# junofficial/mppi_RobotArm

Measured on AMD Instinct MI355X. Metric: MPPI rollouts/sec (K×T state-steps/s) + control-step latency, K=65536 T=64, higher is better.
Workload: dtype f32

## Files before the change

### mppi_robotarm_amd/csrc/mppi_merge.h

```cpp
#pragma once

namespace mppi {


typedef unsigned int u32x2 __attribute__((__vector_size__(2 * sizeof(unsigned int))));
typedef unsigned int u32x4 __attribute__((__vector_size__(4 * sizeof(unsigned int))));
constexpr int kSC1 = 16;

__device__ __forceinline__ __amdgpu_buffer_rsrc_t rows_rsrc(const void* p, int bytes) {
    return __builtin_amdgcn_make_buffer_rsrc(const_cast<void*>(p), 0, bytes, 0x00020000);
}
__device__ __forceinline__ double ld_wt(__amdgpu_buffer_rsrc_t r, int idx) {
    return __builtin_bit_cast(double, __builtin_amdgcn_raw_buffer_load_b64(r, idx * 8, 0, kSC1));
}
__device__ __forceinline__ double ld_prev(__amdgpu_buffer_rsrc_t r, int idx) {
    return __builtin_bit_cast(double, __builtin_amdgcn_raw_buffer_load_b64(r, idx * 8, 0, 0));
}
__device__ __forceinline__ void st_wt(__amdgpu_buffer_rsrc_t r, int idx, double v) {
    __builtin_amdgcn_raw_buffer_store_b64(__builtin_bit_cast(u32x2, v), r, idx * 8, 0, kSC1);
}
constexpr int kOffRange = 1 << 26;

__device__ __forceinline__ void st_gran(__amdgpu_buffer_rsrc_t r, int idx, double v, unsigned tag) {
    const unsigned long long b = (unsigned long long)__double_as_longlong(v);
// ... 124 lines not shown
        } else {
            rho_r = ld_wt(rows, lrow);
            eta_l = ld_wt(rows, lrow + 1);
#pragma unroll
            for (int j = 0; j < LB; ++j) {
                const int i = j / MAXCH, col = tid + (j % MAXCH) * NT;
                v[j] = ld_wt(rows, (i < nr && col < ncol) ? (rb + i) * stride + 1 + col : kOffRange);
            }
        }
        const double rho_l = lane < nr ? rho_r : INFINITY;
        const double rnew = min_raw_f64(rho, wave_min_f64(rho_l));
        double s_l = 0.0;
        if (lane < nr) {
            const double s = exp((rnew - rho_l) * inv_lambda);
            s_l = s >= kMergeFloor ? s : 0.0;
        }
        const unsigned long long rel = __ballot(s_l != 0.0);
        const int nrr = __popcll(rel);
        nrel += nrr;
        if (rnew < rho && rho != INFINITY) {
            const double f = exp((rnew - rho) * inv_lambda);
#pragma unroll
            for (int ch = 0; ch < MAXCH; ++ch) acc[ch] *= f;
            eta *= f;
        }
        rho = rnew;
        if constexpr (EAGER) {
#pragma unroll
            for (int j = 0; j < LB; ++j) {
                const int i = j / MAXCH, ch = j % MAXCH;
                if (i < nr) {
                    const double s = readlane_f64(s_l, i);
                    if (s != 0.0) {
                        acc[ch] = fma(s, v[j], acc[ch]);
                        if (ch == 0) eta = fma(s, readlane_f64(eta_l, i), eta);
                    }
                }
            }
        } else {
            const int krow = lane < nrr ? select_bit(rel, lane) : 0;
            for (int b0 = 0; b0 < nrr; b0 += RB) {
                const bool eta_on = b0 == 0 && lane < nrr;
                const int eidx = eta_on ? (rb + krow) * stride + 1 : kOffRange;
                double x[LB];
                if constexpr (GRAN) {
                    u32x4 ge, gv[LB];
                    for (unsigned spins = 0;; ++spins) {
                        asm volatile("" ::: "memory");
                        ge = ld_gran(rows, eidx);
                        bool ok = !eta_on || gran_ok(ge, tag);
#pragma unroll
                        for (int j = 0; j < LB; ++j) {
                            const int i = b0 + j / MAXCH, col = tid + (j % MAXCH) * NT;
                            const bool on = i < nrr && col < ncol;
                            gv[j] = ld_gran(rows, on ? (rb + __builtin_amdgcn_readlane(krow, i)) * stride + 1 + col
                                                     : kOffRange);
                            ok = ok && (!on || gran_ok(gv[j], tag));
                        }
                        if (__all(ok)) break;
                        MPPI_SPIN_OR_GIVE_UP_L(spins, deadline, tmo, lane, gave_up = true);
                    }
                    if (eta_on) eta_l = gran_val(ge);
#pragma unroll
                    for (int j = 0; j < LB; ++j) x[j] = gran_val(gv[j]);
                } else {
                    if (b0 == 0) eta_l = ld_wt(rows, eidx);
#pragma unroll
                    for (int j = 0; j < LB; ++j) {
                        const int i = b0 + j / MAXCH, col = tid + (j % MAXCH) * NT;
                        x[j] = ld_wt(rows, (i < nrr && col < ncol)
                                               ? (rb + __builtin_amdgcn_readlane(krow, i)) * stride + 1 + col
                                               : kOffRange);
                    }
                }
#pragma unroll
                for (int j = 0; j < LB; ++j) {
                    const int i = b0 + j / MAXCH, ch = j % MAXCH;
                    if (i < nrr) {
                        const double s = readlane_f64(s_l, __builtin_amdgcn_readlane(krow, i));
                        acc[ch] = fma(s, x[j], acc[ch]);
                        if (ch == 0) eta = fma(s, readlane_f64(eta_l, i), eta);
                    }
                }
            }
        }
    }
    if (failed) *failed = __syncthreads_or(gave_up);
    if constexpr (final) {
        put_final<NT, MAXCH>(rho, acc, eta, nrel, geo, sm, out_row, w_eps_out);
    } else {
        auto put = [&](int col, double x) {
            if constexpr (GRAN) st_gran(*out_wt, out_idx * stride + col, x, tag);
            else st_wt(*out_wt, out_idx * stride + col, x);
        };
#pragma unroll
        for (int ch = 0; ch < MAXCH; ++ch) {
            const int col = tid + ch * NT;
            if (col >= ncol) continue;
            if (col == 0) put(0, rho);
            put(1 + col, acc[ch]);
        }
    }
}

template <int NT, int MAXCH, RowsVia VIA, class SM>
__device__ __forceinline__ bool direct_merge(__amdgpu_buffer_rsrc_t rows, int n, const RowGeo& geo,
                                             double inv_lambda, SM& sm, double* out_row, double* w_eps_out,
                                             unsigned tag, unsigned* tmo, unsigned long long* dbg = nullptr,
                                             const double* rho_pre = nullptr) {
    constexpr bool GRAN = VIA == RowsVia::Gran, PRE = VIA == RowsVia::Prev;
    constexpr int P = kDirectRows / 64;
    auto ld = [](__amdgpu_buffer_rsrc_t r, int idx) { return PRE ? ld_prev(r, idx) : ld_wt(r, idx); };
    constexpr int LB = 16;
    constexpr int RB = LB / MAXCH;
    const int tid = threadIdx.x, lane = tid & 63;
    const int stride = geo.stride, ncol = geo.ncol;
    double rho_l[P];
    if constexpr (GRAN) {
        if (tid < 64) {
            u32x4 gr[P];
            for (unsigned spins = 0;; ++spins) {
                asm volatile("" ::: "memory");
                bool ok = true;
#pragma unroll
                for (int j = 0; j < P; ++j) {
                    const int r = lane + 64 * j;
                    gr[j] = ld_gran(rows, r < n ? r * stride : kOffRange);
                    ok = ok && (r >= n || gran_ok(gr[j], tag));
                }
                if (__all(ok)) break;
                MPPI_SPIN_OR_GIVE_UP(spins, tmo, lane);
            }
#pragma unroll
            for (int j = 0; j < P; ++j) sm.rho[lane + 64 * j] = lane + 64 * j < n ? gran_val(gr[j]) : INFINITY;
        }
        __syncthreads();
#pragma unroll
        for (int j = 0; j < P; ++j) rho_l[j] = sm.rho[lane + 64 * j];
    } else if constexpr (PRE) {
#pragma unroll
        for (int j = 0; j < P; ++j) rho_l[j] = rho_pre[j];
    } else {
#pragma unroll
        for (int j = 0; j < P; ++j) {
            const int r = lane + 64 * j;
            const double x = ld_wt(rows, r < n ? r * stride : kOffRange);
            rho_l[j] = r < n ? x : INFINITY;
        }
    }
    double m = rho_l[0];
#pragma unroll
    for (int j = 1; j < P; ++j) m = min_raw_f64(m, rho_l[j]);
    const double rho = wave_min_f64(m);
    double s_l[P];
    unsigned long long rel[P];
    int nrel = 0;
#pragma unroll
    for (int j = 0; j < P; ++j) {
        const double s = exp((rho - rho_l[j]) * inv_lambda);
        s_l[j] = (lane + 64 * j < n && s >= kMergeFloor) ? s : 0.0;
        rel[j] = __ballot(s_l[j] != 0.0);
        nrel += __popcll(rel[j]);
    }
    const int G = MAXCH == 1 ? max(1, NT / ncol) : 1;
    if (nrel > (G > 1 ? min(64, 2 * kDirectMax * G) : kDirectMax)) return false;
    int k = lane, row = 0;
    bool found = false;
#pragma unroll
    for (int j = 0; j < P; ++j) {
        const int cnt = __popcll(rel[j]);
        if (!found && k < cnt) {
            row = 64 * j + select_bit(rel[j], k);
            found = true;
        } else if (!found) {
            k -= cnt;
        }
    }
    double sk = 0.0;
#pragma unroll
    for (int j = 0; j < P; ++j) {
        const double sj = __shfl(s_l[j], row & 63);
        if ((row >> 6) == j) sk = sj;
    }
    const bool mine = lane < nrel;
    STAMP(13, NOW());
    double acc[MAXCH], eta = 0.0, eta_k = 0.0;
#pragma unroll
    for (int ch = 0; ch < MAXCH; ++ch) acc[ch] = 0.0;
    if (G == 1) {
        for (int b0 = 0; b0 < nrel; b0 += RB) {
            double v[LB];
            if constexpr (GRAN) {
                const bool eta_on = b0 == 0 && mine;
                u32x4 ge, gv[LB];
                for (unsigned spins = 0;; ++spins) {
                    asm volatile("" ::: "memory");
                    ge = ld_gran(rows, eta_on ? row * stride + 1 : kOffRange);
                    bool ok = !eta_on || gran_ok(ge, tag);
#pragma unroll
                    for (int j = 0; j < LB; ++j) {
                        const int i = b0 + j / MAXCH, col = tid + (j % MAXCH) * NT;
                        const bool on = i < nrel && col < ncol;
                        gv[j] = ld_gran(rows, on ? __builtin_amdgcn_readlane(row, i) * stride + 1 + col : kOffRange);
                        ok = ok && (!on || gran_ok(gv[j], tag));
                    }
                    if (__all(ok)) break;
                    MPPI_SPIN_OR_GIVE_UP(spins, tmo, lane);
                }
                if (eta_on) eta_k = gran_val(ge);
#pragma unroll
                for (int j = 0; j < LB; ++j) v[j] = gran_val(gv[j]);
            } else {
                if (b0 == 0) eta_k = ld(rows, mine ? row * stride + 1 : kOffRange);
#pragma unroll
                for (int j = 0; j < LB; ++j) {
                    const int i = b0 + j / MAXCH, col = tid + (j % MAXCH) * NT;
                    v[j] = ld(rows, (i < nrel && col < ncol) ? __builtin_amdgcn_readlane(row, i) * stride + 1 + col
                                                              : kOffRange);
                }
            }
#pragma unroll
            for (int j = 0; j < LB; ++j) {
                const int i = b0 + j / MAXCH, ch = j % MAXCH;
                if (i < nrel) {
                    const double s = readlane_f64(sk, i);
                    acc[ch] = fma(s, v[j], acc[ch]);
                    if (ch == 0) eta = fma(s, readlane_f64(eta_k, i), eta);
                }
            }
        }
    } else {
        const int grp = tid / ncol, gcol = tid - grp * ncol;
        const bool active = grp < G;
        for (int b0 = 0; b0 < nrel; b0 += RB * G) {
            double v[LB], sf[LB];
            int roff[LB];
            bool on[LB];
#pragma unroll
            for (int j = 0; j < LB; ++j) {
                const int i = b0 + grp + G * j;
                on[j] = active && i < nrel;
                const int r = __builtin_amdgcn_ds_bpermute(min(i, 63) << 2, row);
                sf[j] = __shfl(sk, min(i, 63));
                roff[j] = on[j] ? r * stride + 1 + gcol : kOffRange;
            }
            if constexpr (GRAN) {
                u32x4 gv[LB];
                for (unsigned spins = 0;; ++spins) {
                    asm volatile("" ::: "memory");
                    bool ok = true;
#pragma unroll
                    for (int j = 0; j < LB; ++j) {
                        gv[j] = ld_gran(rows, roff[j]);
                        ok = ok && (!on[j] || gran_ok(gv[j], tag));
                    }
                    if (__all(ok)) break;
                    MPPI_SPIN_OR_GIVE_UP(spins, tmo, lane);
                }
#pragma unroll
                for (int j = 0; j < LB; ++j) v[j] = gran_val(gv[j]);
            } else {
#pragma unroll
                for (int j = 0; j < LB; ++j) v[j] = ld(rows, roff[j]);
            }
#pragma unroll
            for (int j = 0; j < LB; ++j)
                if (on[j]) acc[0] = fma(sf[j], v[j], acc[0]);
        }
        if (active) sm.part[tid] = acc[0];
        __syncthreads();
        if (grp == 0) {
            double a = sm.part[gcol];
            for (int g = 1; g < G; ++g) a += sm.part[g * ncol + gcol];
            acc[0] = a;
            if (tid == 0) sm.red[0] = a;
        }
        __syncthreads();
        eta = sm.red[0];
    }
    STAMP(14, NOW());
    put_final<NT, MAXCH>(rho, acc, eta, nrel, geo, sm, out_row, w_eps_out);
    return true;
}

__device__ __forceinline__ bool arrive_last(unsigned* counter, unsigned expected, unsigned* s_flag, bool acquire) {
    asm volatile("s_waitcnt vmcnt(0)" ::: "memory");
    __syncthreads();
    if (threadIdx.x == 0) {
        const unsigned prev = __hip_atomic_fetch_add(counter, 1u, __ATOMIC_RELAXED, __HIP_MEMORY_SCOPE_AGENT);
        const bool last = prev == expected - 1;
        if (last) __hip_atomic_store(counter, 0u, __ATOMIC_RELAXED, __HIP_MEMORY_SCOPE_AGENT);
        if (last && acquire) {
            __builtin_amdgcn_fence(__ATOMIC_ACQUIRE, "agent");
            asm volatile("s_waitcnt vmcnt(0)" ::: "memory");
        }
        *s_flag = last ? 1u : 0u;
    }
    __syncthreads();
    return *s_flag != 0;
}

template <int NT, int MAXCH, bool POLL, class SM>
__device__ __forceinline__ bool handoff_merge(__amdgpu_buffer_rsrc_t slab_r, __amdgpu_buffer_rsrc_t gslab_r, int nrows,
                                              const RowGeo& geo, double inv_lambda, SM& sm, unsigned* counters,
                                              bool acquire, unsigned* s_flag, double* partial_out, double* w_eps_out,
                                              unsigned tag, unsigned* epoch, unsigned* tmo, unsigned long long* dbg,
                                              unsigned long long* direct_dbg) {
    constexpr RowsVia VIA = POLL ? RowsVia::Gran : RowsVia::Wt;
    const int ngroups = (nrows + kGroup - 1) / kGroup;
    const int g = blockIdx.x / kGroup;
    const int gsz = min(kGroup, nrows - g * kGroup);
    if constexpr (POLL) {
        if ((int)blockIdx.x != g * kGroup) return false;
        STAMP(3, NOW());
        if (ngroups == 1) {
            merge_rows_block<NT, MAXCH, true, VIA>(slab_r, 0, gsz, geo, inv_lambda, sm, nullptr, 0, partial_out,
                                                   w_eps_out, tag, tmo);
        } else if (blockIdx.x == 0 && nrows <= kDirectRows &&
                   direct_merge<NT, MAXCH, VIA>(slab_r, nrows, geo, inv_lambda, sm, partial_out, w_eps_out, tag, tmo,
                                                direct_dbg)) {
        } else {
            merge_rows_block<NT, MAXCH, false, VIA>(slab_r, g * kGroup, gsz, geo, inv_lambda, sm, &gslab_r, g, nullptr,
                                                    nullptr, tag, tmo);
            STAMP(10, NOW());
            if (blockIdx.x != 0) return false;
            STAMP(4, NOW());
            merge_rows_block<NT, MAXCH, true, VIA>(gslab_r, 0, ngroups, geo, inv_lambda, sm, nullptr, 0, partial_out,
                                                   w_eps_out, tag, tmo);
        }
        if (threadIdx.x == 0) __hip_atomic_store(epoch, tag, __ATOMIC_RELAXED, __HIP_MEMORY_SCOPE_AGENT);
    } else {
        if (!arrive_last(counters + g, (unsigned)gsz, s_flag, acquire)) return false;
        STAMP(3, NOW());
        merge_rows_block<NT, MAXCH, false, VIA>(slab_r, g * kGroup, gsz, geo, inv_lambda, sm, &gslab_r, g, nullptr,
                                                nullptr, 0u, nullptr);
        STAMP(10, NOW());
        if (!arrive_last(counters + ngroups, (unsigned)ngroups, s_flag, acquire)) return false;
        STAMP(4, NOW());
        if (!(ngroups > 1 && nrows <= kDirectRows &&
              direct_merge<NT, MAXCH, VIA>(slab_r, nrows, geo, inv_lambda, sm, partial_out, w_eps_out, 0u, nullptr)))
            merge_rows_block<NT, MAXCH, true, VIA>(gslab_r, 0, ngroups, geo, inv_lambda, sm, nullptr, 0, partial_out,
                                                   w_eps_out, 0u, nullptr);
    }
    return true;
}

template <int NT, class SM>
__device__ __forceinline__ void deferred_merge(__amdgpu_buffer_rsrc_t rows, int n, const RowGeo& geo, double inv_lambda,
                                               SM& sm, int* l_row, double* w_eps_out) {
    constexpr int P = kDirectRows / 64;
    constexpr int LB = 32;
    static_assert(kGroup == 16, "a group is one DPP row of lanes");
    static_assert(kDirectRows / kGroup <= 16, "the group rows merge in one round in either hand-off form");
    const int tid = threadIdx.x, lane = tid & 63;
    const int stride = geo.stride, ncol = geo.ncol;
    double rho_l[P];
#pragma unroll
    for (int j = 0; j < P; ++j) {
        const int r = lane + 64 * j;
        const double x = ld_prev(rows, r < n ? n * stride + r : kOffRange);
        rho_l[j] = r < n ? x : INFINITY;
    }
    if (n > kGroup && direct_merge<NT, 1, RowsVia::Prev>(rows, n, geo, inv_lambda, sm, nullptr, w_eps_out, 0u, nullptr,
                                                           nullptr, rho_l))
        return;
    double rho_g[P], m = INFINITY;
#pragma unroll
    for (int j = 0; j < P; ++j) {
        double v = rho_l[j];
        v = min_raw_f64(v, dpp_f64<0xB1>(v));
        v = min_raw_f64(v, dpp_f64<0x4E>(v));
        v = min_raw_f64(v, dpp_f64<0x141>(v));
        v = min_raw_f64(v, dpp_f64<0x140>(v));
        rho_g[j] = v;
        m = min_raw_f64(m, v);
    }
    const double rho = wave_min_f64(m);
    if (tid < 64) {
        int base = 0;
#pragma unroll
        for (int j = 0; j < P; ++j) {
            const bool in = lane + 64 * j < n;
            const double s1 = exp((rho_g[j] - rho_l[j]) * inv_lambda);
            const double s2 = exp((rho - rho_g[j]) * inv_lambda);
            const bool need = in && s1 >= kMergeFloor && s2 >= kMergeFloor;
            const unsigned long long bal = __ballot(need);
            if (need) {
                const int pos = base + lanes_below(bal);
                l_row[pos] = lane + 64 * j;
                sm.rho[pos] = s1;
                sm.part[pos] = s2;
            }
            base += __popcll(bal);
        }
        if (lane == 0) sm.nrel = base;
    }
    __syncthreads();
    const int nn = sm.nrel;
    double acc = 0.0, accg = 0.0;
    for (int b0 = 0; b0 < nn; b0 += LB) {
        double v[LB];
#pragma unroll
        for (int j = 0; j < LB; ++j) {
            const int i = b0 + j;
            v[j] = ld_prev(rows, (i < nn && tid < ncol) ? l_row[i] * stride + 1 + tid : kOffRange);
        }
#pragma unroll
        for (int j = 0; j < LB; ++j) {
            const int i = b0 + j;
            if (i < nn) {
                accg = fma(sm.rho[i], v[j], accg);
                if (i + 1 == nn || (l_row[i + 1] / kGroup) != (l_row[i] / kGroup)) {
                    acc = fma(sm.part[i], accg, acc);
                    accg = 0.0;
                }
            }
        }
    }
    if (tid == 0) {
        sm.eta = acc;
        sm.rho_fin = rho;
    }
    __syncthreads();
    if (tid >= 1 && tid < ncol) {
        const double w = acc / sm.eta;
        sm.weps[tid - 1] = w;
        if (w_eps_out) w_eps_out[tid - 1] = w;
    }
    __syncthreads();
}

constexpr int kMaxWorld = MPPI_MAX_WORLD;
struct XDesc {
    const void* peer[kMaxWorld];
    double* row;
    unsigned* epoch;
    int rank, world, bytes;
    unsigned timeout_ticks;
};
constexpr unsigned kTmoLocal = 1u, kTmoExchange = 2u, kTmoSplit = 4u;
__device__ __forceinline__ void st_gran_sys(__amdgpu_buffer_rsrc_t r, int idx, double v, unsigned tag) {
    const unsigned long long b = (unsigned long long)__double_as_longlong(v);
    const u32x4 x = {(unsigned)b, tag, (unsigned)(b >> 32), tag};
    __builtin_amdgcn_raw_buffer_store_b128(x, r, idx * 16, 0, kSC1 | 1);
}

template <int NT, int MAXCH, class SM>
__device__ __forceinline__ unsigned exchange_send_merge(const XDesc& x, const RowGeo& geo, double inv_lambda, SM& sm,
                                                        double* w_eps_out, unsigned* tmo) {
    const unsigned tag = (unsigned)__builtin_amdgcn_readfirstlane((int)*x.epoch) + 1u;
    const int par = (int)(tag & 1u), stride = geo.stride;
    for (int idx = threadIdx.x; idx < stride; idx += NT) {
        const double v = x.row[idx];
        for (int p = 0; p < x.world; ++p)
            st_gran_sys(rows_rsrc(x.peer[p], x.bytes), (par * x.world + x.rank) * stride + idx, v, tag);
    }
    bool late = false;
    const unsigned long long dl = x.timeout_ticks ? __builtin_amdgcn_s_memrealtime() + x.timeout_ticks : 0ull;
    merge_rows_block<NT, MAXCH, true, RowsVia::Gran>(rows_rsrc(x.peer[x.rank], x.bytes), par * x.world, x.world, geo,
                                                     inv_lambda, sm, nullptr, 0, nullptr, w_eps_out, tag, nullptr, dl,
                                                     &late);
    late = __syncthreads_or(late || (threadIdx.x == 0 && tmo &&
                                     __hip_atomic_load(tmo, __ATOMIC_RELAXED, __HIP_MEMORY_SCOPE_SYSTEM) != 0u));
    const int sbase = 2 * x.world * stride + par * x.world;
    if ((int)threadIdx.x < x.world)
        st_gran_sys(rows_rsrc(x.peer[threadIdx.x], x.bytes), sbase + x.rank, late ? -1.0 : 1.0, tag);
    return tag;
}

template <int NT>
__device__ __forceinline__ bool exchange_verdict(const XDesc& x, const RowGeo& geo, unsigned tag, unsigned* tmo) {
    const int par = (int)(tag & 1u);
    const int sbase = 2 * x.world * geo.stride + par * x.world;
    const int tid = threadIdx.x, lane = tid & 63;
    bool bad = false, split = false;
    if (tid < 64) {
        const __amdgpu_buffer_rsrc_t own = rows_rsrc(x.peer[x.rank], x.bytes);
        u32x4 g;
        bool missing = false;
        const unsigned long long dl = x.timeout_ticks ? __builtin_amdgcn_s_memrealtime() + x.timeout_ticks : 0ull;
        for (unsigned spins = 0;; ++spins) {
            asm volatile("" ::: "memory");
            g = ld_gran(own, lane < x.world ? sbase + lane : kOffRange);
            if (__all(lane >= x.world || gran_ok(g, tag))) break;
            MPPI_SPIN_OR_GIVE_UP_L(spins, dl, nullptr, lane, missing = true);
        }
        bad = __any(lane < x.world && !(gran_ok(g, tag) && gran_val(g) > 0.0)) || missing;
        split = missing && !__any(lane == x.rank && gran_ok(g, tag) && gran_val(g) < 0.0);
    }
    bad = __syncthreads_or(bad);
    split = __syncthreads_or(split);
    if (tid == 0) {
        if (bad)
            __hip_atomic_store(tmo + 1, split ? kTmoExchange | kTmoSplit : kTmoExchange, __ATOMIC_RELAXED,
                               __HIP_MEMORY_SCOPE_SYSTEM);
        *x.epoch = tag;
    }
    return !bad;
}

}
```

### mppi_robotarm_amd/csrc/mppi_rocm.hip

```cpp
#include <hip/hip_runtime.h>

#include <math.h>
#include <stdint.h>
#include <stdio.h>
#include <stdlib.h>
#include <string.h>

#include <algorithm>
#include <chrono>
#include <string>
#include <type_traits>

#include "mppi_device.h"
#include "mppi_host.h"
#include "mppi_rocm.h"

namespace {

using namespace mppi;

constexpr int kThreads = 256;

struct alignas(16) StepStatic {
    float4 win[kSlots];
// ... 89 lines not shown
}

__device__ __forceinline__ f32x2 splat(float x) { return f32x2{x, x}; }


__device__ __forceinline__ void disc_pair_hits(const ObstR& o, int p, f32x2 cs1, f32x2 cs12, f32x2 fk, bool (&h)[4]) {
    const DiscPair d = load_pair(o, p);
    seg_hits(d.cX, d.cY, cs1, fk.x, d.r2, h[0], h[2]);
    const f32x2 qX = __builtin_elementwise_fma(splat(-fk.x), splat(cs1.x), d.cX);
    const f32x2 qY = __builtin_elementwise_fma(splat(-fk.x), splat(cs1.y), d.cY);
    seg_hits(qX, qY, cs12, fk.y, d.r2, h[1], h[3]);
}

template <int NP>
__device__ __forceinline__ bool obst_any(const ObstR& o, f32x2 cs1, f32x2 cs12, f32x2 fk) {
    bool any = false;
#pragma unroll
    for (int p = 0; p < (NP ? NP : kObstPairs); ++p) {
        if (NP == 0 && 2 * p >= o.n) break;
        bool h[4];
        disc_pair_hits(o, p, cs1, cs12, fk, h);
        any |= (h[0] | h[1]) | (h[2] | h[3]);
    }
    return any;
}

__device__ __forceinline__ unsigned obst_mask(const ObstR& o, f32x2 cs1, f32x2 cs12, f32x2 fk) {
    unsigned m = 0;
#pragma unroll
    for (int p = 0; p < kObstPairs; ++p) {
        if (2 * p >= o.n) break;
        bool h[4];
        disc_pair_hits(o, p, cs1, cs12, fk, h);
#pragma unroll
        for (int b = 0; b < 4; ++b) m |= (h[b] ? 1u : 0u) << (4 * p + b);
    }
    return m;
}

__device__ __forceinline__ f32x2 cossin_rev(float a) { return f32x2{__builtin_amdgcn_cosf(a), __builtin_amdgcn_sinf(a)}; }

__device__ __forceinline__ void arm_init(Arm& x, float4 x0) {
    x.Q = f32x2{x0.x, x0.y} * 0.15915494309189535f;
    x.dq = f32x2{x0.z, x0.w};
    x.cs1 = cossin_rev(x.Q.x);
    x.cs12 = cossin_rev(x.Q.x + x.Q.y);
}

__device__ __forceinline__ f32x2 cos_sin_diff(f32x2 cs1, f32x2 cs12) {
    const f32x2 m = cs12 * splat(cs1.x);
    f32x2 r;
    asm("v_pk_fma_f32 %0, %1, %2, %3 op_sel:[1,1,0] op_sel_hi:[0,1,1] neg_hi:[1,0,0]"
        : "=v"(r) : "v"(cs12), "v"(cs1), "v"(m));
    return r;
}

__device__ __forceinline__ void arm_step(Arm& x, f32x2 v, const DynK& k) {
    const float c1 = x.cs1.x, c12 = x.cs12.x;
    const f32x2 cs2 = cos_sin_diff(x.cs1, x.cs12);
    const float c2 = cs2.x, s2 = cs2.y;
    const f32x2 DM11 = __builtin_elementwise_fma(k.zB, splat(c2), k.DA);
    const float M12 = fmaf(k.ED.x, c2, k.ED.y);
    const float h = k.ED.x * s2;
    const f32x2 w = __builtin_elementwise_fma(k.nQ, splat(c12), __builtin_elementwise_fma(k.nP0, splat(c1), v));
    const float dq1 = x.dq.x, dq2 = x.dq.y;
    const float hd1 = h * dq1;
    const f32x2 r = {fmaf(h * dq2, fmaf(2.f, dq1, dq2), w.x), fmaf(-hd1, dq1, w.y)};
    const float det = fmaf(DM11.y, k.ED.y, -(M12 * M12));
    const float rdet = __builtin_amdgcn_rcpf(det);
    const f32x2 ddq = __builtin_elementwise_fma(splat(-M12), f32x2{r.y, r.x}, DM11 * r) * splat(rdet);
    x.dq = __builtin_elementwise_fma(ddq, splat(k.dt2.x), x.dq);
    x.Q = __builtin_elementwise_fma(x.dq, splat(k.dt2.y), x.Q);
    x.cs1 = cossin_rev(x.Q.x);
    x.cs12 = cossin_rev(x.Q.x + x.Q.y);
}

__device__ __forceinline__ f32x2 arm_fk(const Arm& x, const DynK& k) {
    return __builtin_elementwise_fma(splat(k.fk.x), x.cs1, splat(k.fk.y) * x.cs12);
}

__device__ __forceinline__ float cost_pk(f32x2 e, f32x2 f, f32x2 w01, f32x2 w23) {
    const f32x2 s = __builtin_elementwise_fma(f * w23, f, (e * w01) * e);
    return s.x + s.y;
}

using Scratch = MergeScratch<2 * kMaxT>;

constexpr int kPF = 4;

constexpr unsigned kFlagPending = 1u << 31;

__device__ __forceinline__ double nominal_src(const DevStep* st, int tid, int T) {
    const int t = tid >> 1, src = t + 1 < T ? t + 1 : T - 1;
    return tid < 2 * T ? st->u[src][tid & 1] : 0.0;
}
__device__ __forceinline__ double nominal_first(const DevStep* st, int tid) {
    return tid < 2 ? st->u[0][tid] : 0.0;
}

struct HostOut {
    double* p;
    unsigned seq;
};

template <int NT, bool CLAMP, bool DEFER = false, int UAS = 1>
__device__ void nominal_update_block(DevStep* nxt, const KConst& c, Scratch& sm, double u_src, double u_first,
                                     float* upd, HostOut ho, const ClampK& cl, bool publish = true,
                                     float4* s_ua = nullptr, bool store = true) {
    const int tid = threadIdx.x;
    const int T = c.T;
    if constexpr (!DEFER) store = true;
    if (!store) upd = nullptr;
    if (tid < ((2 * T + 63) & ~63)) {
        const int t = tid >> 1, d = tid & 1;
        const int src = t + 1 < T ? t + 1 : T - 1;
        double un = tid < 2 * T ? u_src + median_at(sm, src, d, T, 2) : 0.0;
        bool clampu = false;
        if constexpr (CLAMP) clampu = cl.mode == 2;
        if (clampu) un = clamp_u(un, cl.u_lo[d], cl.u_hi[d]);
        const double other = dpp_f64<0xB1>(un);
        if ((upd || ho.p) && tid < 2) {
            double u0 = u_first + median_at(sm, 0, d, T, 2);
            if (clampu) u0 = clamp_u(u0, cl.u_lo[d], cl.u_hi[d]);
            if (upd) upd[d] = (float)u0;
            if (ho.p) ho.p[2 + d] = u0;
        }
        if (tid < 2 * T) {
            if (upd && t + 1 < T) upd[2 * (t + 1) + d] = (float)un;
            if (ho.p) ho.p[4 + tid] = un;
            if (store) nxt->u[t][d] = un;
            if (d == 0) {
                const double u0 = un, u1 = other;
                const double g0 = c.gamma * u0, g1 = c.gamma * u1;
                const double a0 = g0 * c.sig_inv[0] + g1 * c.sig_inv[2];
                const double a1 = g0 * c.sig_inv[1] + g1 * c.sig_inv[3];
                const float4 row = make_float4((float)u0, (float)u1, (float)a0, (float)a1);
                if (store) nxt->ua[t] = row;
                if constexpr (DEFER) {
                    s_ua[t * UAS] = row;
                    if (t == T - 1)
                        for (int p = 0; p < kPF; ++p) s_ua[(T + p) * UAS] = row;
                }
            }
        }
    }
    if (ho.p) {
        __threadfence_system();
        if (!publish) return;
        __syncthreads();
        if (tid == 0) __hip_atomic_store(reinterpret_cast<unsigned*>(ho.p), ho.seq, __ATOMIC_RELEASE, __HIP_MEMORY_SCOPE_SYSTEM);
    }
}

template <int NT, bool CLAMP, int UAS = 1>
__device__ __forceinline__ void deferred_finish(const KConst& c, const double* rows, const DevStep* st, DevStep* nxt,
                                                double* w_eps_out, float* upd, const ClampK& cl, Scratch& sm,
                                                int* l_row, float4* s_ua, bool store) {
    const int tid = threadIdx.x;
    const double u_cur = nominal_src(st, tid, c.T), u_first = nominal_first(st, tid);
    const RowGeo geo(2 * c.T);
    deferred_merge<NT>(rows_rsrc(rows, c.nblocks * (geo.stride + 1) * 8), c.nblocks, geo, c.inv_lambda, sm, l_row,
                       store ? w_eps_out : nullptr);
    nominal_update_block<NT, CLAMP, true, UAS>(nxt, c, sm, u_cur, u_first, upd, HostOut{nullptr, 0u}, cl, false, s_ua,
                                               store);
}


template <int LPS, int NT, bool POLL, bool CLAMP, bool OBST, bool DEFER = false, bool MOVE = false>
__global__ __launch_bounds__(NT) void rollout_kernel(
    const KConst c, const StepStatic ss, const DevStep* __restrict__ st, const float2* __restrict__ noise,
    double* __restrict__ S_out, double* __restrict__ slab, double* __restrict__ gslab,
    unsigned* __restrict__ counters, double* __restrict__ partial_out, double* __restrict__ w_eps_out,
    DevStep* __restrict__ nxt, unsigned flags, const XDesc xd, unsigned* __restrict__ epoch, unsigned* __restrict__ tmo,
    float* __restrict__ upd, const HostOut ho, unsigned long long* __restrict__ dbg, const ClampK cl,
    const ObstK ob) {
    static_assert(CLAMP || !OBST, "the OBST kernels are built with CLAMP only");
    static_assert(OBST || !MOVE, "moving discs are discs");
    static_assert(!DEFER || !POLL, "the deferred form leaves plain rows");
    static_assert(!DEFER || NT >= kDirectRows, "s_k holds the deferred merge's row list");
    __shared__ float4 s_win[kSlots];
    constexpr int UAS = MOVE ? 1 + kObstRow : 1;
    __shared__ float4 s_ua[(kMaxT + kPF) * UAS];
    __shared__ double s_redd[NT / 64];
    __shared__ int s_cnt[NT / 64];
    __shared__ int s_k[NT];
    __shared__ double s_e[NT];
    __shared__ unsigned s_flag;
    __shared__ Scratch sm;

    const int tid = threadIdx.x, lane = tid & 63, wave = tid >> 6;
    const int k_raw = (blockIdx.x * NT + tid) / LPS;
    const bool valid = k_raw < c.K_local;
    const int k = valid ? k_raw : c.K_local - 1;
    const float exf = (c.k_offset + k) < c.k_exploit ? 1.f : 0.f;
    const int K = c.K_local, T = c.T;

    STAMP(0, NOW());
#ifdef MPPI_STAMPS
    STAMP(8, (unsigned long long)__builtin_amdgcn_s_getreg(0xF804));
    STAMP(9, (unsigned long long)__builtin_amdgcn_s_getreg(0xF814));
#endif
    const float2* np = noise + k;
    float2 ring[kPF];
#pragma unroll
    for (int j = 0; j < kPF; ++j) ring[j] = np[(size_t)(j < T ? j : T - 1) * K];
    const unsigned tag_v = POLL ? __hip_atomic_load(epoch, __ATOMIC_RELAXED, __HIP_MEMORY_SCOPE_AGENT) + 1u : 0u;
    const double u_cur = (!DEFER && (flags & MPPI_FLAG_FUSED_UPDATE)) ? nominal_src(st, tid, T) : 0.0;
    const double u_first = (!DEFER && (flags & MPPI_FLAG_FUSED_UPDATE)) ? nominal_first(st, tid) : 0.0;
    bool pending = false;
    if constexpr (DEFER) {
        pending = (flags & kFlagPending) != 0;
        if (pending) deferred_finish<NT, CLAMP, UAS>(c, gslab, st, nxt, w_eps_out, upd, cl, sm, s_k, s_ua, blockIdx.x == 0);
        STAMP(10, NOW());
    }
    const float4 wrow = ss.win[tid & (kSlots - 1)];
    Search<LPS> sr;
    sr.load(ss.key, ss.ctr, tid & (LPS - 1));
    Arm x;
    arm_init(x, ss.x0);
    DynK dk = make_dynk(c, sr.cx, sr.cy);
    if constexpr (CLAMP) dynk_limits(dk, cl);
    ObstR od{};
    if constexpr (MOVE) {
        if (tid < T) stage_obst_row(s_ua + tid * UAS + 1, ob, tid);
        od = ObstR{s_ua + 1, __builtin_amdgcn_readfirstlane(ob.n)};
    } else if constexpr (OBST) {
        __shared__ float4 s_obst[2 * kObstPairs];
        if (tid == 0) stage_obst(s_obst, ob);
        od = ObstR{s_obst, __builtin_amdgcn_readfirstlane(ob.n)};
    }
    int hits = 0;
    bool hit_last = false;
    if (!pending)
        for (int i = tid; i < T + kPF; i += NT) s_ua[i * UAS] = st->ua[i < T ? i : T - 1];
    if (tid < kSlots) s_win[tid] = wrow;
    __syncthreads();
    float4 uring[kPF];
#pragma unroll
    for (int j = 0; j < kPF; ++j) uring[j] = s_ua[(j < T ? j : T - 1) * UAS];

    double S = 0.0;
    f32x2 S4 = {0.f, 0.f};
    f32x2 ee = {0.f, 0.f}, ef = {0.f, 0.f};
    float4 pr = make_float4(0.f, 0.f, 0.f, 0.f);
    f32x2 pp = {0.f, 0.f}, pd = {0.f, 0.f};
    auto add_pending = [&]() {
        f32x4 r = {pr.x, pr.y, pr.z, pr.w};
        asm volatile("" : "+v"(r) : "v"(x.cs12));
        ee = pp - f32x2{r.x, r.y};
        ef = pd - f32x2{r.z, r.w};
        S4 = __builtin_elementwise_fma(ef * dk.w23, ef, __builtin_elementwise_fma(ee * dk.w01, ee, S4));
    };
    int ua_off = vgpr_opaque(0);
    auto dstep = [&](int t, auto slot_c, auto h_c, auto np_c) {
        constexpr int slot = decltype(slot_c)::value;
        constexpr int H = decltype(h_c)::value;
        constexpr int NP = decltype(np_c)::value;
        const bool h = H == 2 ? t > 0 : H == 1;
        f32x2 e = {ring[slot].x, ring[slot].y};
        f32x4 ua = {uring[slot].x, uring[slot].y, uring[slot].z, uring[slot].w};
        asm volatile("" : "+v"(e), "+v"(ua));
        f32x2 v = __builtin_elementwise_fma(splat(exf), f32x2{ua.x, ua.y}, e);
        if constexpr (CLAMP) v = clamp_v(v, dk);
        S4 = __builtin_elementwise_fma(f32x2{ua.z, ua.w}, v, S4);
        const int tl = t + kPF < T ? t + kPF : T - 1;
        ring[slot] = np[(size_t)tl * K];
        uring[slot] = *reinterpret_cast<const float4*>(reinterpret_cast<const char*>(s_ua) + ua_off +
                                                       (kPF + slot) * UAS * (int)sizeof(float4));
        if (!MOVE && slot == kPF - 1) ua_off += kPF * UAS * (int)sizeof(float4);
        PIN_LOADS();
        arm_step(x, v, dk);
        if (h) {
            add_pending();
            if (slot == 0) {
                S += (double)(S4.x + S4.y);
                S4 = f32x2{0.f, 0.f};
            }
        }
        if constexpr (OBST) {
            if constexpr (MOVE) {
                const ObstR ot{reinterpret_cast<const float4*>(reinterpret_cast<const char*>(od.rec) + ua_off +
                                                               slot * UAS * (int)sizeof(float4)),
                               od.n};
                hit_last = obst_any<NP>(ot, x.cs1, x.cs12, dk.fk);
                if (slot == kPF - 1) ua_off += kPF * UAS * (int)sizeof(float4);
            } else {
                hit_last = obst_any<NP>(od, x.cs1, x.cs12, dk.fk);
            }
            hits += hit_last ? 1 : 0;
        }
        pp = arm_fk(x, dk);
        pd = x.dq;
        const f32x2 d = pp - dk.ctr;
        pr = s_win[sr.nearest_d(d.x, d.y)];
    };
    using I0 = std::integral_constant<int, 0>;
    using I1 = std::integral_constant<int, 1>;
    using I2 = std::integral_constant<int, 2>;
    using I3 = std::integral_constant<int, 3>;
    using H0 = std::integral_constant<int, 0>;
    using H1 = std::integral_constant<int, 1>;
    using H2 = std::integral_constant<int, 2>;
    static_assert(kPF == 4, "unrolled for a 4-deep ring");
    using NP = std::integral_constant<int, (OBST && LPS == 1) ? kObstPairs : 0>;
    int t = 0;
    STAMP(12, NOW());
    if constexpr (LPS == 1) {
        dstep(0, I0{}, H0{}, NP{});
        for (t = 1; t + kPF <= T; t += kPF) {
            dstep(t, I1{}, H1{}, NP{});
            dstep(t + 1, I2{}, H1{}, NP{});
            dstep(t + 2, I3{}, H1{}, NP{});
            dstep(t + 3, I0{}, H1{}, NP{});
#ifdef MPPI_STAMPS
            if (t == 1) STAMP(13, NOW());
            if (t + kPF == T / 2 + 1) STAMP(14, NOW());
#endif
        }
        if (t < T) dstep(t, I1{}, H1{}, NP{});
        if (t + 1 < T) dstep(t + 1, I2{}, H1{}, NP{});
        if (t + 2 < T) dstep(t + 2, I3{}, H1{}, NP{});
    } else {
        for (; t + kPF <= T; t += kPF) {
            dstep(t, I0{}, H2{}, NP{});
            dstep(t + 1, I1{}, H2{}, NP{});
            dstep(t + 2, I2{}, H2{}, NP{});
            dstep(t + 3, I3{}, H2{}, NP{});
#ifdef MPPI_STAMPS
            if (t == 0) STAMP(13, NOW());
            if (t + kPF == T / 2) STAMP(14, NOW());
#endif
        }
        if (t < T) dstep(t, I0{}, H2{}, NP{});
        if (t + 1 < T) dstep(t + 1, I1{}, H2{}, NP{});
        if (t + 2 < T) dstep(t + 2, I2{}, H2{}, NP{});
    }
    add_pending();
    S += (double)(S4.x + S4.y);
    S += (double)cost_pk(ee, ef, f32x2{arg_f(c.tw[0]), arg_f(c.tw[1])}, f32x2{arg_f(c.tw[2]), arg_f(c.tw[3])});
    if constexpr (OBST) {
        hits += hit_last ? 1 : 0;
        S += ob.w * (double)hits;
    }

    STAMP(1, NOW());
    const bool owner = valid && sr.sub == 0;
    if (S_out && owner) S_out[k] = S;

    const int stride = 2 + 2 * T;
    const RowGeo geo(2 * T);
    const int nrows = c.nblocks;
    const int ngroups = (nrows + kGroup - 1) / kGroup;
    constexpr int kValBytes = POLL ? 16 : 8;
    const __amdgpu_buffer_rsrc_t slab_r = rows_rsrc(slab, nrows * (stride + (DEFER ? 1 : 0)) * kValBytes);
    const __amdgpu_buffer_rsrc_t gslab_r = rows_rsrc(gslab, ngroups * stride * kValBytes);
    const unsigned tag = __builtin_amdgcn_readfirstlane(tag_v);
    auto publish = [&](int idx, double v) {
        if constexpr (POLL) st_gran(slab_r, idx, v, tag);
        else st_wt(slab_r, idx, v);
    };
    const double rho_b = block_min_f64<NT>(owner ? S : INFINITY, sm);
    if (tid == 0) publish(blockIdx.x * stride, rho_b);
    if constexpr (DEFER)
        if (tid == 0) publish(nrows * stride + blockIdx.x, rho_b);
    const LaneWeight lw = block_weigh(owner, S, rho_b, c.inv_lambda, lane, wave, s_cnt, s_redd);
    __syncthreads();
    double eta_b;
    int nl = block_compact<NT>(lw, k, wave, s_cnt, s_redd, s_k, s_e, &eta_b);
    __syncthreads();
    if (tid == 0) publish(blockIdx.x * stride + 1, eta_b);
    STAMP(15, NOW());
    nl = __builtin_amdgcn_readfirstlane(nl);
    if (nl <= kSparseMax) {
        const float* nf = reinterpret_cast<const float*>(noise);
        for (int col = tid; col < 2 * T; col += NT) {
            const float* base = nf + (size_t)(col >> 1) * K * 2 + (col & 1);
            publish(blockIdx.x * stride + 2 + col, gather_col(base, 2, s_k, s_e, nl));
        }
    } else {
        constexpr int NS = NT / LPS;
        constexpr int PER = (NS + 63) / 64;
        constexpr int kRowBatch = 4;
        const int k0 = blockIdx.x * NS;
        double w[PER];
        dense_weights<NT, NS>(lw, k, K, s_e, w);
        for (int tb = wave * kRowBatch; tb < T; tb += (NT / 64) * kRowBatch) {
            float2 e[kRowBatch][PER];
#pragma unroll
            for (int r = 0; r < kRowBatch; ++r) {
                const int tr = min(tb + r, T - 1);
#pragma unroll
                for (int i = 0; i < PER; ++i)
                    e[r][i] = noise[(size_t)tr * K + min(k0 + lane + 64 * i, K - 1)];
            }
#pragma unroll
            for (int r = 0; r < kRowBatch; ++r) {
                double ax = 0.0, ay = 0.0;
#pragma unroll
                for (int i = 0; i < PER; ++i) {
                    ax = fma(w[i], (double)e[r][i].x, ax);
                    ay = fma(w[i], (double)e[r][i].y, ay);
                }
                ax = wave_sum_f64(ax);
                ay = wave_sum_f64(ay);
                if (lane == 0 && tb + r < T) {
                    publish(blockIdx.x * stride + 2 + 2 * (tb + r), ax);
                    publish(blockIdx.x * stride + 3 + 2 * (tb + r), ay);
                }
            }
        }
    }
    STAMP(2, NOW());
    STAMP(5, (unsigned long long)nl);
    if constexpr (DEFER) return;
    if (!handoff_merge<NT, 1, POLL>(slab_r, gslab_r, nrows, geo, c.inv_lambda, sm, counters, c.acquire != 0, &s_flag,
                                    partial_out, w_eps_out, tag, epoch, tmo, dbg, dbg))
        return;
    STAMP(11, NOW());
    STAMP(6, (unsigned long long)sm.nrel);
    if (flags & MPPI_FLAG_EXCHANGE) {
        const unsigned xtag = exchange_send_merge<NT, 1>(xd, geo, c.inv_lambda, sm, w_eps_out, tmo);
        if (flags & MPPI_FLAG_FUSED_UPDATE) nominal_update_block<NT, CLAMP>(nxt, c, sm, u_cur, u_first, upd, ho, cl, false);
        exchange_verdict<NT>(xd, geo, xtag, tmo);
        if ((flags & MPPI_FLAG_FUSED_UPDATE) && ho.p && threadIdx.x == 0)
            __hip_atomic_store(reinterpret_cast<unsigned*>(ho.p), ho.seq, __ATOMIC_RELEASE, __HIP_MEMORY_SCOPE_SYSTEM);
    } else if (flags & MPPI_FLAG_FUSED_UPDATE) {
        nominal_update_block<NT, CLAMP>(nxt, c, sm, u_cur, u_first, upd, ho, cl);
    }
    STAMP(7, NOW());
}

template <int NT, bool CLAMP>
__global__ __launch_bounds__(NT) void merge_kernel(const KConst c, const double* parts, int n, double* w_eps_out,
                                                   const DevStep* cur, DevStep* nxt, unsigned flags, float* upd,
                                                   const HostOut ho, const ClampK cl) {
    __shared__ Scratch sm;
    const int tid = threadIdx.x;
    const double u_cur = (flags & MPPI_FLAG_FUSED_UPDATE) ? nominal_src(cur, tid, c.T) : 0.0;
    const double u_first = (flags & MPPI_FLAG_FUSED_UPDATE) ? nominal_first(cur, tid) : 0.0;
    const __amdgpu_buffer_rsrc_t r = rows_rsrc(parts, n * (2 + 2 * c.T) * 8);
    merge_rows_block<NT, 1, true, RowsVia::Wt>(r, 0, n, RowGeo(2 * c.T), c.inv_lambda, sm, nullptr, 0, nullptr,
                                               w_eps_out, 0u, nullptr);
    if (flags & MPPI_FLAG_FUSED_UPDATE) nominal_update_block<NT, CLAMP>(nxt, c, sm, u_cur, u_first, upd, ho, cl);
}

template <int NT, bool CLAMP>
__global__ __launch_bounds__(NT) void finalize_kernel(const KConst c, const double* rows, const DevStep* cur,
                                                      DevStep* nxt, double* w_eps_out, float* upd, const ClampK cl) {
    __shared__ Scratch sm;
    __shared__ int s_row[kDirectRows];
    __shared__ float4 s_ua[kMaxT + kPF];
    deferred_finish<NT, CLAMP>(c, rows, cur, nxt, w_eps_out, upd, cl, sm, s_row, s_ua, true);
}

constexpr int kTrajTB = 8;
template <bool NOISE, bool CLAMP>
__global__ __launch_bounds__(kThreads) void traj_kernel(const KConst c, const StepStatic ss,
                                                        const float2* __restrict__ base, int bstride,
                                                        const float2* __restrict__ noise, int Kn,
                                                        float4* __restrict__ out, const ClampK cl) {
    __shared__ float4 tile[kTrajTB][kThreads];
    const int tid = threadIdx.x;
    const int k0 = blockIdx.x * kThreads;
    const int k = min(k0 + tid, Kn - 1);
    const int nk = min(kThreads, Kn - k0);
    const int T = c.T;
    const float exf = NOISE ? ((c.k_offset + k) < c.k_exploit ? 1.f : 0.f) : 1.f;
    Arm x;
    arm_init(x, ss.x0);
    DynK dk = make_dynk(c, 0.f, 0.f);
    if constexpr (CLAMP) dynk_limits(dk, cl);
    auto load_tile = [&](int t0, float2 (&d)[kTrajTB]) {
#pragma unroll
        for (int j = 0; j < kTrajTB; ++j) {
            const int t = min(t0 + j, T - 1);
            const int ti = t == 0 ? T - 1 : t - 1;
            d[j] = NOISE ? noise[(size_t)ti * c.K_local + k] : make_float2(0.f, 0.f);
        }
    };
    auto tile_steps = [&](const float2 (&cur)[kTrajTB], int t0) {
        const int nt = min(kTrajTB, T - t0);
#pragma unroll
        for (int j = 0; j < kTrajTB; ++j) {
            if (j >= nt) break;
            const int t = t0 + j;
            const int ti = t == 0 ? T - 1 : t - 1;
            const float2 b = base[ti * bstride];
            f32x2 v = {b.x, b.y};
            if (NOISE) v = __builtin_elementwise_fma(splat(exf), v, f32x2{cur[j].x, cur[j].y});
            if constexpr (CLAMP) v = clamp_v(v, dk);
            arm_step(x, v, dk);
            const f32x2 q = x.Q * 6.283185307179586f;
            tile[j][tid] = make_float4(q.x, q.y, x.dq.x, x.dq.y);
        }
        __syncthreads();
        for (int i = tid; i < nk * nt; i += kThreads) {
            const int s = i / nt, j = i - s * nt;
            out[(size_t)(k0 + s) * T + t0 + j] = tile[j][s];
        }
        __syncthreads();
    };
    float2 ta[kTrajTB], tb[kTrajTB], tc[kTrajTB];
    load_tile(0, ta);
    load_tile(kTrajTB, tb);
    for (int t0 = 0; t0 < T; t0 += 3 * kTrajTB) {
        load_tile(t0 + 2 * kTrajTB, tc);
        tile_steps(ta, t0);
        if (t0 + kTrajTB >= T) break;
        load_tile(t0 + 3 * kTrajTB, ta);
        tile_steps(tb, t0 + kTrajTB);
        if (t0 + 2 * kTrajTB >= T) break;
        load_tile(t0 + 4 * kTrajTB, tb);
        tile_steps(tc, t0 + 2 * kTrajTB);
    }
}

__global__ __launch_bounds__(kThreads) void nearest_debug_kernel(const KConst c, const StepStatic ss,
                                                                 const DevStep* __restrict__ st,
                                                                 const float2* __restrict__ noise, int Kn,
                                                                 int* __restrict__ slot, float2* __restrict__ pos,
                                                                 const ClampK cl) {
    const int k = blockIdx.x * kThreads + threadIdx.x;
    if (k >= Kn) return;
    const int T = c.T;
    const float exf = (c.k_offset + k) < c.k_exploit ? 1.f : 0.f;
    Search<1> sr;
    sr.load(ss.key, ss.ctr, 0);
    Arm x;
    arm_init(x, ss.x0);
    DynK dk = make_dynk(c, sr.cx, sr.cy);
    dynk_limits(dk, cl);
    const bool clampv = cl.mode != 0;
    for (int t = 0; t < T; ++t) {
        const float4 ua = st->ua[t];
        const float2 e = noise[(size_t)t * c.K_local + k];
        f32x2 v = __builtin_elementwise_fma(splat(exf), f32x2{ua.x, ua.y}, f32x2{e.x, e.y});
        if (clampv) v = clamp_v(v, dk);
        arm_step(x, v, dk);
        const f32x2 p = arm_fk(x, dk);
        const f32x2 d = p - dk.ctr;
        slot[(size_t)k * T + t] = (int)sr.nearest_d(d.x, d.y);
        pos[(size_t)k * T + t] = make_float2(p.x, p.y);
    }
}

__global__ __launch_bounds__(kThreads) void obstacle_debug_kernel(const KConst c, const StepStatic ss,
                                                                  const DevStep* __restrict__ st,
                                                                  const float2* __restrict__ noise, int Kn,
                                                                  unsigned* __restrict__ mask, float4* __restrict__ dir,
                                                                  const ClampK cl, const ObstK ob) {
    const int k = blockIdx.x * kThreads + threadIdx.x;
    const int T = c.T;
    const float exf = (c.k_offset + k) < c.k_exploit ? 1.f : 0.f;
    Arm x;
    arm_init(x, ss.x0);
    DynK dk = make_dynk(c, 0.f, 0.f);
    dynk_limits(dk, cl);
    __shared__ float4 s_obst[kMaxT * kObstRow];
    if ((int)threadIdx.x < T) stage_obst_row(s_obst + threadIdx.x * kObstRow, ob, threadIdx.x);
    __syncthreads();
    const int nd = __builtin_amdgcn_readfirstlane(ob.n);
    if (k >= Kn) return;
    for (int t = 0; t < T; ++t) {
        const float4 ua = st->ua[t];
        const float2 e = noise[(size_t)t * c.K_local + k];
        f32x2 v = __builtin_elementwise_fma(splat(exf), f32x2{ua.x, ua.y}, f32x2{e.x, e.y});
        v = clamp_v(v, dk);
        arm_step(x, v, dk);
        mask[(size_t)k * T + t] = obst_mask(ObstR{s_obst + t * kObstRow, nd}, x.cs1, x.cs12, dk.fk);
        dir[(size_t)k * T + t] = make_float4(x.cs1.x, x.cs1.y, x.cs12.x, x.cs12.y);
    }
}

__global__ __launch_bounds__(kThreads) void philox_noise_kernel(int K_local, int T, long long k_offset,
                                                                unsigned long long seed,
                                                                unsigned long long step, float L00,
                                                                float L10, float L11, float2* out) {
    const int k = (int)blockIdx.x * kThreads + (int)threadIdx.x;
    if (k >= K_local) return;
    const int t0 = 2 * (int)blockIdx.y;
    const unsigned long long kg = (unsigned long long)(k_offset + k);
    const uint4 ctr = make_uint4((unsigned)kg, (unsigned)(kg >> 32), (unsigned)t0, (unsigned)step);
    const uint2 key = make_uint2((unsigned)seed, (unsigned)(seed >> 32) ^ (unsigned)(step >> 32));
    const uint4 r = philox4x32_10(ctr, key);
    const float2 za = box_muller(r.x, r.y), zb = box_muller(r.z, r.w);
    const float z0 = za.x, z1 = za.y, z2 = zb.x, z3 = zb.y;
    out[(size_t)t0 * K_local + k] = make_float2(L00 * z0, fmaf(L10, z0, L11 * z1));
    if (t0 + 1 < T) out[(size_t)(t0 + 1) * K_local + k] = make_float2(L00 * z2, fmaf(L10, z2, L11 * z3));
}

}


struct mppi_ctx {
    mppi_config cfg;
    int device = 0;
    hipStream_t stream = nullptr;
    int lps = 1, nt = 256, nblocks = 0;
    KConst kc;
    ClampK ck{};
    ObstK ok{};
    StepStatic stat{};
    mppi_host::DevBuf<DevStep> d_step;
    int cur = 0;
    mppi_host::DevBuf<double> d_drows;
// ... 749 lines not shown
```

Before: 168.1 billion.

## Hoist deferred-finish loads ahead of window loads and add candidate-first direct merge

Splits the deferred finish into a load phase (nominal controls and per-block rho values) that is issued before the window/search loads, so those global loads overlap rather than serialize at kernel start. It also adds a PRE-path in direct_merge that selects candidate rows by exponent threshold and issues the row-value loads before computing exp weights, to hide load latency behind the exp evaluation. The new path falls back to the old code if any candidate falls below the merge floor, and it adds register pressure from the prefetched value arrays.

```diff
diff --git a/mppi_robotarm_amd/csrc/mppi_merge.h b/mppi_robotarm_amd/csrc/mppi_merge.h
--- a/mppi_robotarm_amd/csrc/mppi_merge.h
+++ b/mppi_robotarm_amd/csrc/mppi_merge.h
@@ -300,6 +300,126 @@
 #pragma unroll
     for (int j = 1; j < P; ++j) m = min_raw_f64(m, rho_l[j]);
     const double rho = wave_min_f64(m);
+    if constexpr (PRE) {
+        static_assert(!PRE || MAXCH == 1, "the deferred finish merges one column chunk");
+        const int Gc = max(1, NT / ncol);
+        double x_l[P];
+        unsigned long long cand[P];
+        bool is[P];
+        int ncand = 0;
+#pragma unroll
+        for (int j = 0; j < P; ++j) {
+            x_l[j] = (rho - rho_l[j]) * inv_lambda;
+            is[j] = lane + 64 * j < n && x_l[j] >= -45.0;
+            cand[j] = __ballot(is[j]);
+            ncand += __popcll(cand[j]);
+        }
+        if (ncand <= (Gc > 1 ? min(64, 2 * kDirectMax * Gc) : kDirectMax)) {
+            int row = 0, base = 0;
+#pragma unroll
+            for (int j = 0; j < P; ++j) {
+                const int cnt = __popcll(cand[j]);
+                const int below = lanes_below(cand[j]);
+                const int dst = base + (is[j] ? below : cnt + lane - below);
+                const int got = __builtin_amdgcn_ds_permute((dst & 63) << 2, lane + 64 * j);
+                if (lane >= base && lane < base + cnt) row = got;
+                base += cnt;
+            }
+            const bool mine = lane < ncand;
+            STAMP(13, NOW());
+            if (Gc == 1) {
+                double v[LB];
+                double eta_k = ld_prev(rows, mine ? row * stride + 1 : kOffRange);
+#pragma unroll
+                for (int j = 0; j < LB; ++j)
+                    v[j] = ld_prev(rows, (j < ncand && tid < ncol) ? __builtin_amdgcn_readlane(row, j) * stride + 1 + tid
+                                                                   : kOffRange);
+                double xk = 0.0;
+#pragma unroll
+                for (int j = 0; j < P; ++j) {
+                    const double xj = __shfl(x_l[j], row & 63);
+                    if ((row >> 6) == j) xk = xj;
+                }
+                asm volatile("" : "+v"(xk) : : "memory");
+                const double s = exp(xk);
+                const double sk = (mine && s >= kMergeFloor) ? s : 0.0;
+                const int nrel = __popcll(__ballot(sk != 0.0));
+                if (nrel == ncand) {
+                    double acc[MAXCH] = {0.0}, eta = 0.0;
+#pragma unroll
+                    for (int j = 0; j < LB; ++j) {
+                        if (j < nrel) {
+                            const double sj = readlane_f64(sk, j);
+                            acc[0] = fma(sj, v[j], acc[0]);
+                            eta = fma(sj, readlane_f64(eta_k, j), eta);
+                        }
+                    }
+                    STAMP(14, NOW());
+                    put_final<NT, MAXCH>(rho, acc, eta, nrel, geo, sm, out_row, w_eps_out);
+                    return true;
+                }
+            } else {
+                const int grp = tid / ncol, gcol = tid - grp * ncol;
+                const bool active = grp < Gc;
+                const bool two = ncand > RB * Gc;
+                double v0[LB], v1[LB];
+#pragma unroll
+                for (int j = 0; j < LB; ++j) {
+                    const int i = grp + Gc * j;
+                    const int r = __builtin_amdgcn_ds_bpermute(min(i, 63) << 2, row);
+                    v0[j] = ld_prev(rows, (active && i < ncand) ? r * stride + 1 + gcol : kOffRange);
+                }
+                if (two) {
+#pragma unroll
+                    for (int j = 0; j < LB; ++j) {
+                        const int i = RB * Gc + grp + Gc * j;
+                        const int r = __builtin_amdgcn_ds_bpermute(min(i, 63) << 2, row);
+                        v1[j] = ld_prev(rows, (active && i < ncand) ? r * stride + 1 + gcol : kOffRange);
+                    }
+                }
+                double xk = 0.0;
+#pragma unroll
+                for (int j = 0; j < P; ++j) {
+                    const double xj = __shfl(x_l[j], row & 63);
+                    if ((row >> 6) == j) xk = xj;
+                }
+                asm volatile("" : "+v"(xk) : : "memory");
+                const double s = exp(xk);
+                const double sk = (mine && s >= kMergeFloor) ? s : 0.0;
+                const int nrel = __popcll(__ballot(sk != 0.0));
+                if (nrel == ncand) {
+                    double acc[MAXCH] = {0.0};
+#pragma unroll
+                    for (int j = 0; j < LB; ++j) {
+                        const int i = grp + Gc * j;
+                        const double sf = __shfl(sk, min(i, 63));
+                        if (active && i < nrel) acc[0] = fma(sf, v0[j], acc[0]);
+                    }
+                    if (two) {
+#pragma unroll
+                        for (int j = 0; j < LB; ++j) {
+                            const int i = RB * Gc + grp + Gc * j;
+                            const double sf = __shfl(sk, min(i, 63));
+                            if (active && i < nrel) acc[0] = fma(sf, v1[j], acc[0]);
+                        }
+                    }
+                    if (active) sm.part[tid] = acc[0];
+                    __syncthreads();
+                    if (grp == 0) {
+                        double a = sm.part[gcol];
+                        for (int g = 1; g < Gc; ++g) a += sm.part[g * ncol + gcol];
+                        acc[0] = a;
+                        if (tid == 0) sm.red[0] = a;
+                    }
+                    __syncthreads();
+                    const double eta = sm.red[0];
+                    STAMP(14, NOW());
+                    put_final<NT, MAXCH>(rho, acc, eta, nrel, geo, sm, out_row, w_eps_out);
+                    return true;
+                }
+            }
+        }
+    }
     double s_l[P];
     unsigned long long rel[P];
     int nrel = 0;
@@ -493,9 +613,19 @@
     return true;
 }
 
+__device__ __forceinline__ void deferred_rho_loads(__amdgpu_buffer_rsrc_t rows, int n, const RowGeo& geo,
+                                                   double (&rho_raw)[kDirectRows / 64]) {
+    const int lane = threadIdx.x & 63;
+#pragma unroll
+    for (int j = 0; j < kDirectRows / 64; ++j) {
+        const int r = lane + 64 * j;
+        rho_raw[j] = ld_prev(rows, r < n ? n * geo.stride + r : kOffRange);
+    }
+}
 template <int NT, class SM>
 __device__ __forceinline__ void deferred_merge(__amdgpu_buffer_rsrc_t rows, int n, const RowGeo& geo, double inv_lambda,
-                                               SM& sm, int* l_row, double* w_eps_out) {
+                                               SM& sm, int* l_row, double* w_eps_out,
+                                               const double (&rho_raw)[kDirectRows / 64]) {
     constexpr int P = kDirectRows / 64;
     constexpr int LB = 32;
     static_assert(kGroup == 16, "a group is one DPP row of lanes");
@@ -504,11 +634,7 @@
     const int stride = geo.stride, ncol = geo.ncol;
     double rho_l[P];
 #pragma unroll
-    for (int j = 0; j < P; ++j) {
-        const int r = lane + 64 * j;
-        const double x = ld_prev(rows, r < n ? n * stride + r : kOffRange);
-        rho_l[j] = r < n ? x : INFINITY;
-    }
+    for (int j = 0; j < P; ++j) rho_l[j] = lane + 64 * j < n ? rho_raw[j] : INFINITY;
     if (n > kGroup && direct_merge<NT, 1, RowsVia::Prev>(rows, n, geo, inv_lambda, sm, nullptr, w_eps_out, 0u, nullptr,
                                                            nullptr, rho_l))
         return;
diff --git a/mppi_robotarm_amd/csrc/mppi_rocm.hip b/mppi_robotarm_amd/csrc/mppi_rocm.hip
--- a/mppi_robotarm_amd/csrc/mppi_rocm.hip
+++ b/mppi_robotarm_amd/csrc/mppi_rocm.hip
@@ -265,17 +265,28 @@
     }
 }
 
+struct FinishLoads {
+    double u_cur, u_first, rho[kDirectRows / 64];
+};
+__device__ __forceinline__ __amdgpu_buffer_rsrc_t finish_rsrc(const KConst& c, const double* rows) {
+    return rows_rsrc(rows, c.nblocks * (RowGeo(2 * c.T).stride + 1) * 8);
+}
+__device__ __forceinline__ FinishLoads deferred_finish_loads(const KConst& c, const double* rows, const DevStep* st) {
+    const int tid = threadIdx.x;
+    FinishLoads f;
+    f.u_cur = nominal_src(st, tid, c.T);
+    f.u_first = nominal_first(st, tid);
+    deferred_rho_loads(finish_rsrc(c, rows), c.nblocks, RowGeo(2 * c.T), f.rho);
+    return f;
+}
 template <int NT, bool CLAMP, int UAS = 1>
-__device__ __forceinline__ void deferred_finish(const KConst& c, const double* rows, const DevStep* st, DevStep* nxt,
+__device__ __forceinline__ void deferred_finish(const KConst& c, const double* rows, const FinishLoads& f, DevStep* nxt,
                                                 double* w_eps_out, float* upd, const ClampK& cl, Scratch& sm,
                                                 int* l_row, float4* s_ua, bool store) {
-    const int tid = threadIdx.x;
-    const double u_cur = nominal_src(st, tid, c.T), u_first = nominal_first(st, tid);
     const RowGeo geo(2 * c.T);
-    deferred_merge<NT>(rows_rsrc(rows, c.nblocks * (geo.stride + 1) * 8), c.nblocks, geo, c.inv_lambda, sm, l_row,
-                       store ? w_eps_out : nullptr);
-    nominal_update_block<NT, CLAMP, true, UAS>(nxt, c, sm, u_cur, u_first, upd, HostOut{nullptr, 0u}, cl, false, s_ua,
-                                               store);
+    deferred_merge<NT>(finish_rsrc(c, rows), c.nblocks, geo, c.inv_lambda, sm, l_row, store ? w_eps_out : nullptr, f.rho);
+    nominal_update_block<NT, CLAMP, true, UAS>(nxt, c, sm, f.u_cur, f.u_first, upd, HostOut{nullptr, 0u}, cl, false,
+                                               s_ua, store);
 }
 
 
@@ -321,14 +332,31 @@
     const double u_cur = (!DEFER && (flags & MPPI_FLAG_FUSED_UPDATE)) ? nominal_src(st, tid, T) : 0.0;
     const double u_first = (!DEFER && (flags & MPPI_FLAG_FUSED_UPDATE)) ? nominal_first(st, tid) : 0.0;
     bool pending = false;
+    float4 wrow;
+    Search<LPS> sr;
+    auto window_loads = [&]() {
+        wrow = ss.win[tid & (kSlots - 1)];
+        sr.load(ss.key, ss.ctr, tid & (LPS - 1));
+    };
     if constexpr (DEFER) {
         pending = (flags & kFlagPending) != 0;
-        if (pending) deferred_finish<NT, CLAMP, UAS>(c, gslab, st, nxt, w_eps_out, upd, cl, sm, s_k, s_ua, blockIdx.x == 0);
+        if constexpr (!MOVE) {
+            FinishLoads fl;
+            if (pending) fl = deferred_finish_loads(c, gslab, st);
+            PIN_LOADS();
+            window_loads();
+            PIN_LOADS();
+            if (pending) deferred_finish<NT, CLAMP, UAS>(c, gslab, fl, nxt, w_eps_out, upd, cl, sm, s_k, s_ua, blockIdx.x == 0);
+        } else {
+            if (pending)
+                deferred_finish<NT, CLAMP, UAS>(c, gslab, deferred_finish_loads(c, gslab, st), nxt, w_eps_out, upd, cl, sm,
+                                                s_k, s_ua, blockIdx.x == 0);
+            window_loads();
+        }
         STAMP(10, NOW());
-    }
-    const float4 wrow = ss.win[tid & (kSlots - 1)];
-    Search<LPS> sr;
-    sr.load(ss.key, ss.ctr, tid & (LPS - 1));
+    } else {
+        window_loads();
+    }
     Arm x;
     arm_init(x, ss.x0);
     DynK dk = make_dynk(c, sr.cx, sr.cy);
@@ -563,7 +591,8 @@
     __shared__ Scratch sm;
     __shared__ int s_row[kDirectRows];
     __shared__ float4 s_ua[kMaxT + kPF];
-    deferred_finish<NT, CLAMP>(c, rows, cur, nxt, w_eps_out, upd, cl, sm, s_row, s_ua, true);
+    deferred_finish<NT, CLAMP>(c, rows, deferred_finish_loads(c, rows, cur), nxt, w_eps_out, upd, cl, sm, s_row, s_ua,
+                               true);
 }
 
 constexpr int kTrajTB = 8;
```

Result: slower. 164.7 billion (-2.0%).
